# vita-epfl/CrowdNav

Measured on AMD Instinct MI355X. Metric: env-steps/sec (whole node), 4096 envs x 5 humans, ORCA step, higher is better.
Workload: dtype f32 ORCA solve + f64 env step

## Files before the change

### crowdnav_amd/csrc/crowdnav_amd.hip

```cpp
#include "engine_host.h"
#include "rollout_fused.h"
#include "records_kernels.h"

thread_local char cn_g_err[512] = "";

void cn_launch_orca(cn_engine* e, float* out_vel) {
    pick_maxl(e, [&](auto maxl) {
        pick_bool(e->P.kd, [&](auto kd) {
            hipLaunchKernelGGL((cn::orca_kernel<decltype(maxl)::value, decltype(kd)::value>), dim3(grid_envs(e)), dim3(e->P.threads),
                               e->smem, e->stream, e->P, e->S, out_vel);
        });
    });
}

extern "C" {

const char* cn_last_error(void) { return cn_g_err; }
int cn_abi_version(void) { return CN_ABI_VERSION; }

static bool headline_geometry(const cn::Params& P) {
    return P.A == 6 && P.NC == 5 && P.E == 2 && P.nA == 12 && P.pairs == 60 && P.threads == 64;
}

int cn_create(const cn_config* c, cn_engine** out) {
// ... 28 lines not shown
        return fail(CN_ERR_NO_DEVICE, "no HIP device visible: the MI355X engine has no CPU fallback");
    if (c->device < 0 || c->device >= ndev) return fail(CN_ERR_INVALID, "device %d out of range", c->device);
    CN_HIP(hipSetDevice(c->device));

    cn_engine* e = new (std::nothrow) cn_engine();
    if (!e) return fail(CN_ERR_INVALID, "out of host memory");
    e->cfg = *c;
    e->stream = nullptr;
    e->io_valid = false;
    e->steps_since_fill = -1;
    e->sarl = nullptr;
    e->orca_fresh = false;
    e->async_fill = false;
    e->rollout_done = nullptr;
    e->next_fill_stream = 0;
    for (int i = 0; i < cn_engine::kFillStreams; ++i) e->fill_streams[i] = nullptr;
    for (uint64_t& c : e->launch_counts) c = 0;
    cn::Params& P = e->P;
    P.B = c->num_envs;
    P.A = c->num_humans + 1;
    P.NC = P.A - 1;
    const int e_max = cn::kWave / P.A;
    const bool small_lp = (P.NC < c->max_neighbors ? P.NC : c->max_neighbors) <= 5;
    int e_want = env_int("CROWDNAV_AMD_ENVS_PER_WAVE", small_lp ? (P.B > 2048 ? 2 : 1) : (P.B + 4095) / 4096);
    P.E = e_want < 1 ? 1 : (e_want > e_max ? e_max : e_want);
    int w_want = env_int("CROWDNAV_AMD_WAVES_PER_BLOCK", 1);
    const int w_useful = (P.E * P.A * P.NC + cn::kWave - 1) / cn::kWave;
    if (w_want > w_useful) w_want = w_useful;
    if (w_want > cn::kMaxBlock / cn::kWave) w_want = cn::kMaxBlock / cn::kWave;
    P.threads = cn::kWave * (w_want < 1 ? 1 : w_want);
    P.nA = P.E * P.A;
    P.pairs = P.nA * P.NC;
    P.ring_depth = env_int("CROWDNAV_AMD_RING_DEPTH", 48);
    if (P.ring_depth < 1) P.ring_depth = 1;
    e->maxl = ((P.NC < c->max_neighbors ? P.NC : c->max_neighbors) <= 5) ? 5 : 10;
    P.kd = P.A > cn::kKdLeaf ? 1 : 0;
    P.sched = -1;
    e->sched_min = env_int("CROWDNAV_AMD_SCHED_MIN_STEPS", 24);
    e->sched_force = env_int("CROWDNAV_AMD_SCHED_FORCE", 0) != 0;
    e->sched_reserve = env_int("CROWDNAV_AMD_DYN_RESERVE", 0);
    e->sched_dynamic = env_int("CROWDNAV_AMD_SCHED_DYNAMIC", 1) != 0;
    e->scenario_cache = env_int("CROWDNAV_AMD_SCENARIO_CACHE", 1) != 0;
    e->dyn_visits = env_int("CROWDNAV_AMD_DYN_VISITS", 0);
    P.dyn_visits = 3;
    {
        hipDeviceProp_t prop;
        const bool ok = hipGetDeviceProperties(&prop, c->device) == hipSuccess && prop.multiProcessorCount > 0;
        e->sched_slots = 12 * (ok ? prop.multiProcessorCount : 256);
    }
    P.kdl = cn::kd_layout(P.nA, P.A, P.E);
    e->smem = cn::smem_bytes(P.nA, P.pairs, e->maxl, P.A, P.E);
    e->use_fused = env_int("CROWDNAV_AMD_FUSED", 1) != 0;
    e->fused_split = env_int("CROWDNAV_AMD_FUSED_SPLIT", 1);
    e->split_slots = 0;
    if (headline_geometry(P)) {
        int per_cu = 0;
        hipDeviceProp_t prop;
        if (hipOccupancyMaxActiveBlocksPerMultiprocessor(&per_cu, cn::rollout_fused_kernel<true, true>, 2 * cn::kWave, e->smem) == hipSuccess &&
            hipGetDeviceProperties(&prop, c->device) == hipSuccess && prop.multiProcessorCount > 0)
            e->split_slots = per_cu * prop.multiProcessorCount;
    }
    e->gen_wave = env_int("CROWDNAV_AMD_WAVE_SCENARIOS", c->num_humans > 8 ? 1 : 0) != 0;
    P.robot_visible = c->robot_visible ? 1 : 0;
    P.robot_orca = c->robot_policy == CN_ROBOT_ORCA;
    P.robot_unicycle = c->robot_kinematics == CN_UNICYCLE;
    e->async_fill = (c->flags & CN_FLAG_ASYNC_SCENARIO_FILL) != 0 && e->gen_wave;
    P.async_fill = e->async_fill ? 1 : 0;
    if (e->async_fill && !getenv("CROWDNAV_AMD_RING_DEPTH")) P.ring_depth = 144;
    e->fill_queue_wgs = env_int("CROWDNAV_AMD_FILL_QUEUE_WGS", 1024);
    P.dt = c->time_step;
    P.time_limit = c->time_limit;
    P.success_reward = c->success_reward;
    P.collision_penalty = c->collision_penalty;
    P.discomfort_dist = c->discomfort_dist;
    P.discomfort_factor = c->discomfort_penalty_factor;
    P.robot_safety = c->robot_safety_space;
    P.human_safety = c->human_safety_space;
    P.orca.neighbor_dist = (float)c->neighbor_dist;
    P.orca.inv_time_horizon = 1.0f / (float)c->time_horizon;
    P.orca.inv_time_step = 1.0f / (float)c->time_step;
    P.orca.max_neighbors = c->max_neighbors;
    e->C.num_agents = P.A;
    e->C.rule = c->scenario_rule;
    e->C.randomize = c->randomize_attributes ? 1 : 0;
    e->C.circle_radius = c->circle_radius;
    e->C.square_width = c->square_width;
    e->C.discomfort_dist = c->discomfort_dist;
    e->C.human_radius = c->human_radius;
    e->C.human_v_pref = c->human_v_pref;
    e->C.robot_radius = c->robot_radius;
    e->C.robot_v_pref = c->robot_v_pref;
    int cap_log2 = env_int("CROWDNAV_AMD_MAX_ATTEMPTS_LOG2", c->num_humans > 8 ? 23 : 20);
    if (cap_log2 < 6) cap_log2 = 6;
    if (cap_log2 > 40) cap_log2 = 40;
    e->C.max_attempts = 1ull << cap_log2;
    e->C.error = nullptr;

    const size_t n = (size_t)P.B * P.A;
    int rc = CN_OK;
    cn::StateView& S = e->S;
    if ((rc = dev_alloc(e, &S.pos, n)) || (rc = dev_alloc(e, &S.vel, n)) || (rc = dev_alloc(e, &S.goal, n)) ||
        (rc = dev_alloc(e, &S.rv, n)) || (rc = dev_alloc(e, &S.gtime, (size_t)P.B)) ||
        (rc = dev_alloc(e, &S.theta, (size_t)P.B)) ||
        (rc = dev_alloc(e, &S.rsim_radius, n)) || (rc = dev_alloc(e, &S.rsim_max_speed, (size_t)P.B)) ||
        (rc = dev_alloc(e, &S.rsim_valid, (size_t)P.B)) || (rc = dev_alloc(e, &S.mt_key, (size_t)624 * P.B)) ||
        (rc = dev_alloc(e, &S.mt_pos, (size_t)P.B)) || (rc = dev_alloc(e, &e->probe_key, (size_t)624)) ||
        (rc = dev_alloc(e, &S.ring_pos, n * P.ring_depth)) || (rc = dev_alloc(e, &S.ring_goal, n * P.ring_depth)) ||
        (rc = dev_alloc(e, &S.ring_rv, n * P.ring_depth)) ||
        (rc = dev_alloc(e, &S.ring_mt_key, e->gen_wave ? (size_t)64 : (size_t)624 * cn::kRedoLanes)) ||
        (rc = dev_alloc(e, &S.redo_list, e->gen_wave ? (size_t)1 : (size_t)P.B * P.ring_depth)) ||
        (rc = dev_alloc(e, &S.redo_count, (size_t)1)) ||
// ... 341 lines not shown
        } else {
            hipLaunchKernelGGL(cn::ring_fill_wave_async_kernel, dim3(e->P.B * e->P.ring_depth), dim3(cn::kWave), 0, fs, e->P, e->C,
                               e->S, R);
        }
        e->launch_counts[CN_COUNT_ASYNC_FILLS] += 1;
        e->steps_since_fill = 0;
        return CN_OK;
    }
    if (e->steps_since_fill >= 0 && e->steps_since_fill + n_steps <= e->P.ring_depth) {
        e->steps_since_fill += n_steps;
        return CN_OK;
    }
    const int fill_lanes = e->P.B * e->P.ring_depth;
    const dim3 fill_grid((fill_lanes + cn::kWave - 1) / cn::kWave);
    if (e->gen_wave) {
        hipLaunchKernelGGL(cn::ring_fill_wave_kernel, dim3(fill_lanes), dim3(cn::kWave), 0, e->stream, e->P, e->C, e->S, R);
    } else {
        CN_HIP(hipMemsetAsync(e->S.redo_count, 0, sizeof(int), e->stream));
        hipLaunchKernelGGL(cn::ring_fill_kernel, fill_grid, dim3(cn::kWave), 0, e->stream, e->P, e->C, e->S, R);
        hipLaunchKernelGGL(cn::ring_redo_kernel, dim3(cn::kRedoLanes / cn::kWave), dim3(cn::kWave), 0, e->stream, e->P, e->C,
                           e->S);
    }
    std::swap(e->S.ring_filled_in, e->S.ring_filled_out);
    e->launch_counts[CN_COUNT_RING_FILLS] += 1;
    e->steps_since_fill = n_steps;
    return CN_OK;
}

static int rollout_route(const cn_engine* e, const double* action) {
    const cn::Params& P = e->P;
    static const bool use_geom20 = env_int("CROWDNAV_AMD_GEOM20", 1) != 0;
    if (e->use_fused && !e->async_fill && e->maxl == 5 && !P.robot_unicycle && P.NC <= cn::kFusedMaxNC && P.pairs <= cn::kWave &&
        P.nA * 5 <= cn::kWave && P.threads == cn::kWave) {
#if defined(CN_PHASE_TIMING) || defined(CN_WAVE_TRACE)
        (void)action;
        return CN_ROUTE_FUSED;
#else
        const bool split = e->fused_split != 0 && headline_geometry(P) && P.robot_orca && action == nullptr &&
                           (grid_envs(e) <= e->split_slots || e->fused_split == 2);
        return split ? CN_ROUTE_FUSED_SPLIT : CN_ROUTE_FUSED;
#endif
    }
    if (use_geom20 && e->maxl == 10 && !P.robot_unicycle && P.A == 21 && P.NC == 20 && P.E == 1 && P.threads == 64 &&
        P.orca.max_neighbors == 10 && P.kd)
        return CN_ROUTE_SHARD;
    return CN_ROUTE_GENERIC;
}

static void launch_rollout(cn_engine* e, const cn::RolloutView& R, int n_steps, const double* action) {
    const cn::Params& P = e->P;
    const uint64_t kernels_before = e->launch_counts[CN_COUNT_ROLLOUT_KERNELS];
    const int route = rollout_route(e, action);
    if (route == CN_ROUTE_FUSED_SPLIT) {
        hipLaunchKernelGGL((cn::rollout_fused_kernel<true, true>), dim3(grid_envs(e)), dim3(2 * cn::kWave), e->smem, e->stream, e->P,
                           (const cn::StateView*)e->S_dev, (const int*)e->S.ring_filled_in, R, n_steps, action);
    } else if (route == CN_ROUTE_FUSED) {
        if (headline_geometry(P))
            hipLaunchKernelGGL((cn::rollout_fused_kernel<true>), dim3(grid_envs(e)), dim3(64), e->smem, e->stream, e->P,
                               (const cn::StateView*)e->S_dev, (const int*)e->S.ring_filled_in, R, n_steps, action);
        else
            hipLaunchKernelGGL((cn::rollout_fused_kernel<false>), dim3(grid_envs(e)), dim3(64), e->smem, e->stream, e->P,
                               (const cn::StateView*)e->S_dev, (const int*)e->S.ring_filled_in, R, n_steps, action);
    } else if (route == CN_ROUTE_SHARD) {
        const size_t smem20 = cn::smem_bytes_compact(P.nA, P.pairs, P.A, P.E);
        cn::Params Pk = e->P;
        Pk.sched = -1;
        const int slots = e->sched_slots;
        {
            const bool use_dynamic = e->sched_dynamic;
            const int reserve = e->async_fill ? e->sched_reserve : 0;
            const int G = P.B < slots - reserve ? P.B : slots - reserve;
            int visits = e->dyn_visits > 0 ? e->dyn_visits : (n_steps + 28) / 56;
            if (visits < 3) visits = 3;
            if (visits > n_steps) visits = n_steps;
            Pk.dyn_visits = visits;
            const bool helps = e->sched_force || e->async_fill || P.B > G;
            if (use_dynamic && G > 0 && n_steps >= e->sched_min && action == nullptr && helps && !e->io_host.summary &&
                !e->io_host.blocks) {
                (void)hipMemsetAsync(e->S.dyn_queue, 0, sizeof(int) * ((size_t)P.B + 1), e->stream);
                Pk.sched = cn::kSchedDynamic;
                e->launch_counts[CN_COUNT_ROLLOUT_KERNELS] += 1;
                e->launch_counts[CN_COUNT_SCHEDULED_KERNELS] += 1;
                hipLaunchKernelGGL((cn::rollout_kernel<10, false, true, true>), dim3(G), dim3(64), smem20, e->stream, Pk,
                                   (const cn::StateView*)e->S_dev, (const int*)e->S.ring_filled_in, R, n_steps, action);
                return;
            }
        }
        const int rounds_plain = (P.B + slots - 1) / slots, rounds_sched = (P.B / 4 * 3 + slots - 1) / slots;
        const bool sched = P.B % 4 == 0 && n_steps >= (e->sched_min > 48 ? e->sched_min : 48) && action == nullptr &&
                           (e->sched_force || 4 * rounds_sched < 3 * rounds_plain);
        const int q = sched ? n_steps / 3 : 0, rest = n_steps - 3 * q;
        e->launch_counts[CN_COUNT_ROLLOUT_KERNELS] += (rest > 0 ? 1 : 0) + (q > 0 ? 4 : 0);
        e->launch_counts[CN_COUNT_SCHEDULED_KERNELS] += q > 0 ? 4 : 0;
        if (rest > 0)
            hipLaunchKernelGGL((cn::rollout_kernel<10, false, true, true>), dim3(grid_envs(e)), dim3(64), smem20, e->stream, Pk,
                               (const cn::StateView*)e->S_dev, (const int*)e->S.ring_filled_in, R, rest, action);
        for (int k = 0; k < 4 && q > 0; ++k) {
            Pk.sched = k;
            hipLaunchKernelGGL((cn::rollout_kernel<10, false, true, true>), dim3(P.B / 4 * 3), dim3(64), smem20, e->stream, Pk,
                               (const cn::StateView*)e->S_dev, (const int*)e->S.ring_filled_in, R, q, action);
        }
    } else {
        pick_maxl_uni_kd(e, [&](auto maxl, auto uni, auto kd) {
            hipLaunchKernelGGL((cn::rollout_kernel<decltype(maxl)::value, decltype(uni)::value, false, decltype(kd)::value>),
                               dim3(grid_envs(e)), dim3(e->P.threads), e->smem, e->stream, e->P, (const cn::StateView*)e->S_dev,
                               (const int*)e->S.ring_filled_in, R, n_steps, action);
        });
    }
// ... 140 lines not shown
        return a;
    }();
    return &api;
}
constexpr int kNcclFloat64 = 8;
}

int cn_gather_records(cn_engine* e, void* rccl_comm, int n_ranks, int max_records, const double* blocks,
                      double* blocks_all) {
    int rc = bind(e);
    if (rc) return rc;
    if (!rccl_comm || n_ranks < 1 || max_records < 1 || !blocks || !blocks_all)
        return fail(CN_ERR_INVALID, "cn_gather_records: bad arguments");
    const RcclApi* api = rccl_api();
    if (!api->ok) return fail(CN_ERR_UNSUPPORTED, "cn_gather_records: librccl.so.1 could not be loaded");
    const size_t n = (size_t)e->P.B * cn::record_block_doubles(max_records);
    const int st = api->all_gather(blocks, blocks_all, n, kNcclFloat64, rccl_comm, e->stream);
    if (st) return fail(CN_ERR_HIP, "cn_gather_records: RCCL error %d (%s)", st, api->error_string(st));
    return CN_OK;
}

int cn_mt_random(cn_engine* e, uint32_t seed, int n, double* out) {
    int rc = bind(e);
    if (rc) return rc;
    if (n < 0 || !out) return fail(CN_ERR_INVALID, "cn_mt_random: bad arguments");
    hipLaunchKernelGGL(cn::mt_probe_kernel, dim3(1), dim3(1), 0, e->stream, e->probe_key, seed, n, out);
    CN_HIP(hipGetLastError());
    return CN_OK;
}

}

#ifdef CN_PHASE_TIMING
extern "C" int cn_debug_phase_cycles(unsigned long long* out16, int reset) {
    if (out16 && hipMemcpyFromSymbol(out16, HIP_SYMBOL(cn::cn_phase_cycles), 16 * sizeof(unsigned long long)) != hipSuccess) return -1;
    if (reset) {
        unsigned long long zero[16] = {};
        zero[13] = ~0ull;
        if (hipMemcpyToSymbol(HIP_SYMBOL(cn::cn_phase_cycles), zero, sizeof(zero)) != hipSuccess) return -1;
    }
    return 0;
}
#endif
#ifdef CN_PHASE_TIMING
extern "C" int cn_debug_lazy_counts(unsigned long long* out8, int reset) {
    if (out8 && hipMemcpyFromSymbol(out8, HIP_SYMBOL(cn::cn_lazy_counts), 16 * sizeof(unsigned long long)) != hipSuccess) return -1;
    if (reset) {
        unsigned long long zero[16] = {};
        if (hipMemcpyToSymbol(HIP_SYMBOL(cn::cn_lazy_counts), zero, sizeof(zero)) != hipSuccess) return -1;
    }
    return 0;
}
#endif
#ifdef CN_WAVE_TRACE
extern "C" int cn_debug_wave_trace(unsigned long long* out, int waves) {
    if (waves > 8192) waves = 8192;
    return hipMemcpyFromSymbol(out, HIP_SYMBOL(cn::cn_wave_trace), (size_t)waves * 6 * sizeof(unsigned long long)) == hipSuccess ? 0 : -1;
}
#endif
```

### crowdnav_amd/csrc/engine_host.h

```cpp
#pragma once
#include <hip/hip_runtime.h>

#include <cmath>
#include <cstdarg>
#include <cstdio>
#include <cstdlib>
#include <cstring>
#include <dlfcn.h>
#include <new>
#include <type_traits>
#include <utility>
#include <vector>

#include "../../include/crowdnav_amd.h"
#include "step_kernels.h"



extern thread_local char cn_g_err[512];

namespace {

[[maybe_unused]] int fail(int code, const char* fmt, ...) {
    va_list ap;
    va_start(ap, fmt);
    vsnprintf(cn_g_err, sizeof(cn_g_err), fmt, ap);
    va_end(ap);
    return code;
}

#define CN_HIP(call)                                                                              \
    do {                                                                                          \
        hipError_t err__ = (call);                                                                \
        if (err__ != hipSuccess)                                                                  \
            return fail(CN_ERR_HIP, "%s failed: %s (%s:%d)", #call, hipGetErrorString(err__), __FILE__, \
                        __LINE__);                                                                \
    } while (0)

}

struct cn_engine {
    cn_config cfg;
    cn::Params P;
    cn::ScenarioCfg C;
    cn::StateView S;
    hipStream_t stream;
    cn_rollout_io io_host;
    cn_rollout_io* io_dev;
    cn::StateView* S_dev;
    static constexpr int kFillStreams = 8;
    bool async_fill;
    hipStream_t fill_streams[kFillStreams];
    int* fill_list = nullptr;
    int fill_queue_wgs = 0;
    hipEvent_t rollout_done;
    int next_fill_stream;
    bool io_valid;
    bool rollout_begun = false;
    uint32_t begin_seed_base = 0, begin_seed_mod = 0;
    int steps_since_fill;
    struct cn_sarl* sarl;
    bool orca_fresh;
    double* discount;
    int discount_len;
    uint32_t* probe_key;
    double* summary_scratch;
    int maxl;
    bool gen_wave;
    size_t smem;
    int sched_min, sched_slots, sched_reserve, dyn_visits;
    bool sched_force, sched_dynamic;
    bool use_fused;
    int fused_split;
    int split_slots;
    bool scenario_cache;
    uint64_t launch_counts[CN_LAUNCH_COUNTERS];
    struct Slab {
        char* base;
        size_t size, used;
    };
    std::vector<Slab> slabs;
    struct AllocMark {
        std::vector<size_t> used;
    };
    AllocMark alloc_mark() const {
        AllocMark m;
        for (const Slab& s : slabs) m.used.push_back(s.used);
        return m;
    }
    void alloc_rollback(const AllocMark& m) {
        while (slabs.size() > m.used.size()) {
            (void)hipFree(slabs.back().base);
            slabs.pop_back();
        }
        for (size_t i = 0; i < slabs.size(); ++i) slabs[i].used = m.used[i];
    }
};

namespace {

constexpr size_t kSlabBytes = (size_t)32 << 20, kSlabAlign = 4096;

template <typename T>
int dev_alloc(cn_engine* e, T** out, size_t n) {
    const size_t bytes = (n * sizeof(T) + kSlabAlign - 1) / kSlabAlign * kSlabAlign;
    size_t k = 0;
    while (k < e->slabs.size() && e->slabs[k].used + bytes > e->slabs[k].size) ++k;
    if (k == e->slabs.size()) {
        const size_t size = bytes > kSlabBytes ? (bytes + ((size_t)2 << 20) - 1) >> 21 << 21 : kSlabBytes;
        void* p = nullptr;
        CN_HIP(hipMalloc(&p, size));
        e->slabs.push_back({static_cast<char*>(p), size, 0});
    }
    cn_engine::Slab& sl = e->slabs[k];
    void* p = sl.base + sl.used;
    sl.used += bytes;
    CN_HIP(hipMemset(p, 0, bytes));
    *out = static_cast<T*>(p);
    return CN_OK;
}

[[maybe_unused]] int bind(cn_engine* e) {
    if (!e) return fail(CN_ERR_INVALID, "engine is NULL");
    e->orca_fresh = false;
    CN_HIP(hipSetDevice(e->cfg.device));
    return CN_OK;
// ... 36 lines not shown
```

### crowdnav_amd/csrc/rollout_fused.h

```cpp
#pragma once
#include "step_kernels.h"

namespace cn {

constexpr int kFusedMaxNC = 5;

struct EpisodeRegs {
    double gtime;
    int state, ep_count, ring_filled;
};

template <typename T>
__device__ __forceinline__ T in_vgpr(T x) {
    asm volatile("" : "+v"(x));
    return x;
}

__device__ __forceinline__ void stage_agent(const Params& P, const Smem& s, const Lane& L, const AgentRegs& r,
                                            double human_safety) {
    if (L.lane >= P.nA) return;
    s.kin[L.lane] = make_float4((float)r.px, (float)r.py, (float)r.vx, (float)r.vy);
    s.posd[L.lane] = make_double2(r.px, r.py);
    s.rad[L.lane] = r.rad;
    s.hview[L.lane] = (float)(r.rad + 0.01 + human_safety);
// ... 34 lines not shown
        pr.my_slot = (int)((pr.row_slots >> (8 * c)) & 0xffull);
    }
    return pr;
}

template <typename Mid>
__device__ __forceinline__ void fused_pair_phase(const Params& P, const Smem& s, const PairRow& pr, float range_sq, Mid&& mid) {
    const int my_info = pr.my_info, my_slot = pr.my_slot;
    const unsigned long long row_slots = pr.row_slots;
    const int q = my_info & 0xff, c = (my_info >> 16) & 0xff;
    const int ol = (my_info >> 8) & 0xff;
    const bool robot_sim = (my_info >> 25) & 1;
    const float4 me = s.kin[q];
    const float4 other = s.kin[my_slot];
    float4 ot[kFusedMaxNC];
#pragma unroll
    for (int k = 0; k < kFusedMaxNC; ++k) ot[k] = s.kin[(int)((row_slots >> (8 * k)) & 0xffull)];
    const float* view = robot_sim ? s.rview : s.hview;
    const float rsum = view[q] + view[ol];
    const float odx = me.x - other.x, ody = me.y - other.y;
    const float mine = odx * odx + ody * ody;
    int rank = 0, within = 0;
    {
        const uint32_t mb = __float_as_uint(mine), rb = __float_as_uint(range_sq);
        uint32_t before = 0u, inside = 0u;
#pragma unroll
        for (int k = 0; k < kFusedMaxNC; ++k) {
            const float dx = me.x - ot[k].x, dy = me.y - ot[k].y;
            const uint32_t vb = __float_as_uint(dx * dx + dy * dy);
            const uint32_t tie = (uint32_t)(k - c) >> 31;
            before = __builtin_amdgcn_alignbit(before, vb - mb - tie, 31);
            inside = __builtin_amdgcn_alignbit(inside, vb - rb, 31);
        }
        within = __popc(inside);
        rank = __popc(before & inside);
    }
    mid();
    if (c == 0) s.count[q] = within < P.orca.max_neighbors ? within : P.orca.max_neighbors;
    if (mine < range_sq && rank < P.orca.max_neighbors)
        s.lines[q * kLineStride + rank] =
            make_half_plane(P.orca, me.x, me.y, me.z, me.w, other.x, other.y, other.z, other.w, rsum);
}

template <int MAXL>
__device__ __forceinline__ void fused_candidates(const Params& P, const Smem& s, int lane) {
    if (lane < P.nA * MAXL) {
        const int q = lane / MAXL, k = lane - q * MAXL;
        const float4 so = s.sol[q];
        const float4* lq = s.lines + q * kLineStride;
        s.cand2[q * kLineStride + k] = lp_line_candidate_pairs5(lq, k, lane, so.z, so.x, so.y);
    }
}

template <int MAXL, int BASE_PRIO = 0>
__device__ __forceinline__ bool fused_solve(const Params& P, const Smem& s, int lane, bool solve, float& rx, float& ry,
                                            PhaseClock* clk) {
    (void)P, (void)clk;
    rx = 0.0f, ry = 0.0f;
    int n = 0, fail = 0;
    if (solve) {
        n = s.count[lane];
        const float4 start = s.res[lane];
        rx = start.x, ry = start.y;
        fail = lp_planar_scan<MAXL>(s.lines + lane * kLineStride, s.cand2 + lane * kLineStride, n, rx, ry);
    }
    CN_TICK(clk, 3);
    const bool need = solve && fail < n;
    const unsigned long long nm = __ballot(need);
#ifdef CN_PHASE_TIMING
    if (clk) clk->acc[9] += __popcll(nm);
#endif
    if (nm == 0ull) __builtin_amdgcn_s_setprio(BASE_PRIO);
    if (nm != 0ull) {
        __builtin_amdgcn_s_setprio(3);
        constexpr int kPairs = MAXL * (MAXL - 1) / 2;
        const int n_todo = __popcll(nm);
        bool one_pass_done = false;
        if (n_todo * kPairs <= kWave) {
            const int t = lane / kPairs, m = lane - t * kPairs;
            int a = 0;
            unsigned long long rest = nm;
#pragma unroll
            for (int u = 0; u < kWave / kPairs; ++u) {
                const int bit = rest ? __ffsll((long long)rest) - 1 : 0;
                a = (u == t) ? bit : a;
                rest &= rest - 1ull;
            }
            const bool item = lane < n_todo * kPairs;
            const int i = lp3_program_of(m), base = i * (i - 1) / 2;
            const float4* la = s.lines + a * kLineStride;
            const float4 li = la[i], lj = la[m - base];
            const float radius = s.sol[a].z;
            const float4 pr = lp3_project(li, lj);
            if (item) s.proj[a * kLineStride + m] = pr;
            CN_FUSED_SYNC();
            if (item) {
                const float4* pa = s.proj + a * kLineStride + base;
                s.cand3[a * kLineStride + m] = lp_line_candidate<MAXL - 2>(pa[m - base], pa, m - base, radius, -li.w, li.z, true);
            }
            CN_FUSED_SYNC();
            if (item && m == base)
                s.cand2[a * kLineStride + i] = lp3_inner_program(s.proj + a * kLineStride, s.cand3 + a * kLineStride, i, li, radius);
            CN_FUSED_SYNC();
            if (need)
                lp3_outer_scan(s.lines + lane * kLineStride, s.cand2 + lane * kLineStride, n, fail, s.sol[lane].z, rx, ry);
            one_pass_done = true;
        } else {
            if (need) s.todo[__popcll(nm & ((1ull << lane) - 1ull))] = lane;
            CN_FUSED_SYNC();
            const int items = n_todo * kPairs;
            for (int p = lane; p < items; p += kWave) {
                const int t = p / kPairs, m = p - t * kPairs;
                const int a = s.todo[t];
                const int i = lp3_program_of(m), j = m - i * (i - 1) / 2;
                const float4* la = s.lines + a * kLineStride;
                s.proj[a * kLineStride + m] = lp3_project(la[i], la[j]);
            }
            CN_FUSED_SYNC();
            for (int p = lane; p < items; p += kWave) {
                const int t = p / kPairs, m = p - t * kPairs;
                const int a = s.todo[t];
                const int i = lp3_program_of(m), base = i * (i - 1) / 2;
                const float4 li = s.lines[a * kLineStride + i];
                const float4* pa = s.proj + a * kLineStride + base;
                s.cand3[a * kLineStride + m] = lp_line_candidate<MAXL - 2>(pa[m - base], pa, m - base, s.sol[a].z, -li.w, li.z, true);
            }
            CN_FUSED_SYNC();
        }
        if (need && !one_pass_done)
            lp3_scan(s.lines + lane * kLineStride, s.proj + lane * kLineStride, s.cand3 + lane * kLineStride, n,
                     fail, s.sol[lane].z, rx, ry);
    }
    return nm != 0ull;
}

struct StepConsts {
    double dt, limit, limit1, success, collision, ddist, dfactor, hsafety;
};
__device__ __forceinline__ StepConsts step_consts(const Params& P) {
    StepConsts K;
    K.dt = in_vgpr(P.dt), K.limit = in_vgpr(P.time_limit), K.limit1 = in_vgpr(P.time_limit - 1.0);
    K.success = in_vgpr(P.success_reward), K.collision = in_vgpr(P.collision_penalty);
    K.ddist = in_vgpr(P.discomfort_dist), K.dfactor = in_vgpr(P.discomfort_factor);
    K.hsafety = in_vgpr(P.human_safety);
    return K;
}

__device__ __forceinline__ double swept_distance(const AgentRegs& r, bool human, double2 rp, double act_x, double act_y,
                                                 double new_vx, double new_vy, double dt, double robot_rad) {
    const double x1 = r.px - rp.x, y1 = r.py - rp.y;
    const double wx = r.vx - act_x, wy = r.vy - act_y;
    const double x2 = x1 + wx * dt, y2 = y1 + wy * dt;
    const double sx = x2 - x1, sy = y2 - y1;
    double u = ((0.0 - x1) * sx + (0.0 - y1) * sy) / (sx * sx + sy * sy);
    u = (u > 1.0) ? 1.0 : ((u < 0.0) ? 0.0 : u);
    const bool degenerate = (sx == 0.0 && sy == 0.0);
    const double cx = degenerate ? 0.0 - x1 : (x1 + u * sx) - 0.0;
    const double cy = degenerate ? 0.0 - y1 : (y1 + u * sy) - 0.0;
    const double endx = r.px + new_vx * dt, endy = r.py + new_vy * dt;
    const double d = norm2(human ? cx : endx - r.gx, human ? cy : endy - r.gy);
    return human ? d - r.rad - robot_rad : d;
}

struct StepOutcome {
    double reward, dmin;
    int info;
    bool done;
};
__device__ __forceinline__ StepOutcome reduce_env(const Params& P, const Smem& s, int ebase, double gtime, const StepConsts& K) {
    const double goal_dist = s.closest[ebase];
    const double robot_rad = s.rad[ebase];
    double dmin = std::numeric_limits<double>::infinity();
    bool collision = false;
    for (int i = 1; i < P.A; ++i) {
        const double c = s.closest[ebase + i];
        const bool hit = c < 0.0;
        dmin = (!collision & !hit & (c < dmin)) ? c : dmin;
        collision = collision | hit;
    }
    const bool timeout = gtime >= K.limit1;
    const bool reaching = goal_dist < robot_rad;
    const bool danger = dmin < K.ddist;
    double reward = danger ? (dmin - K.ddist) * K.dfactor * K.dt : 0.0;
    int info = danger ? CN_DANGER : CN_NOTHING;
    reward = reaching ? K.success : reward, info = reaching ? CN_REACH_GOAL : info;
    reward = collision ? K.collision : reward, info = collision ? CN_COLLISION : info;
    reward = timeout ? 0.0 : reward, info = timeout ? CN_TIMEOUT : info;
    const bool done = timeout | collision | reaching;
    return StepOutcome{reward, dmin, info, done};
}

__device__ __forceinline__ void write_record(const cn_rollout_io& io, int env, int ep_count, int info, int cur_steps,
                                             double cur_return, double time, int cur_danger, double cur_dsum) {
    if (io.record_capacity > 0) {
        const size_t k = (size_t)env * io.record_capacity + (ep_count % io.record_capacity);
        if (io.ep_outcome) io.ep_outcome[k] = (uint8_t)info;
        if (io.ep_steps) io.ep_steps[k] = cur_steps;
        if (io.ep_return) io.ep_return[k] = cur_return;
        if (io.ep_time) io.ep_time[k] = time;
        if (io.ep_danger) io.ep_danger[k] = cur_danger;
        if (io.ep_danger_dmin_sum) io.ep_danger_dmin_sum[k] = cur_dsum;
    }
}

#ifdef CN_WAVE_TRACE
static __device__ unsigned long long cn_wave_trace[8192 * 6];
#endif

constexpr int kSplitOrcaPrio = 1;
__device__ __forceinline__ void split_barrier() {
    asm volatile("s_waitcnt lgkmcnt(0)\n\ts_barrier" ::: "memory");
}

template <int MAXL>
__device__ __forceinline__ void split_orca_wave(const Params& P, const Smem& s, int n_steps) {
    const int lane = (int)threadIdx.x - kWave;
    float2* const vel = reinterpret_cast<float2*>(s.act);
    const float range_sq = P.orca.neighbor_dist * P.orca.neighbor_dist;
    const double c_dt = in_vgpr(P.dt);
    split_barrier();
    __builtin_amdgcn_s_setprio(kSplitOrcaPrio);
    const PairRow pr = pair_row_of(P, s, lane);
    double px = 0.0, py = 0.0;
    float rx = 0.0f, ry = 0.0f;
    bool solved = false;
    for (int u = 0;;) {
        split_barrier();
        const bool ended = __builtin_amdgcn_readfirstlane(s.flag[0]) != 0;
        if (!ended) ++u;
        if (u >= n_steps) {
            split_barrier();
            break;
        }
        if (lane < P.nA) {
            if (ended) {
                const double2 p = s.posd[lane];
                px = p.x, py = p.y;
            } else if (solved) {
                px = px + (double)rx * c_dt;
                py = py + (double)ry * c_dt;
                s.kin[lane] = make_float4((float)px, (float)py, rx, ry);
            }
        }
        CN_FUSED_SYNC();
        if (lane < P.pairs) fused_pair_phase(P, s, pr, range_sq, [] {});
        split_barrier();
        fused_candidates<MAXL>(P, s, lane);
        CN_FUSED_SYNC();
        solved = lane < P.nA && s.sol[lane < P.nA ? lane : 0].w != 0.0f;
        fused_solve<MAXL, kSplitOrcaPrio>(P, s, lane, solved, rx, ry, nullptr);
        if (lane < P.nA) vel[lane] = make_float2(rx, ry);
    }
}

template <bool HEADLINE, bool SPLIT = false>
__global__ __launch_bounds__((SPLIT ? 2 : 1) * kWave, (SPLIT ? 4 : HEADLINE ? 3 : 1)) void rollout_fused_kernel(
    Params P_in, const StateView* Sd, const int* ring_filled_in, RolloutView R, int n_steps, const double* ext_action) {
    static_assert(HEADLINE || !SPLIT, "the two-wave kernel exists for the headline geometry only");
#ifdef CN_WAVE_TRACE
    const unsigned long long wt_entry = __builtin_amdgcn_s_memrealtime();
    unsigned long long wt_fallbacks = 0ull, wt_ends = 0ull;
#endif
    constexpr int MAXL = 5;
    Params P = P_in;
    if (HEADLINE) {
        P.A = 6, P.NC = 5, P.E = 2, P.nA = 12, P.pairs = 60, P.threads = 64;
    }
    const Smem s = carve<MAXL>(P);
    if constexpr (SPLIT) {
        if (__builtin_amdgcn_readfirstlane((int)threadIdx.x) >= kWave) {
            split_orca_wave<MAXL>(P, s, n_steps);
            return;
        }
    }
    const Lane L = lane_of(P);
    AgentRegs r = {};
    float robot_max_speed = 0.0f;
    const bool robot = L.valid && L.a == 0;
    const cn_rollout_io* iop = R.io;
    double theta = 0.0;
    EpisodeRegs ep{0.0, kRetired, 0, 0};
    double cur_return = 0.0, cur_dsum = 0.0;
    int cur_steps = 0, cur_danger = 0;
    {
        const StateView S = *Sd;
        const cn_rollout_io io = *iop;
        const size_t gi = L.valid ? L.gi : 0;
        const int env = L.valid ? L.env : 0;
        const double2 p0 = S.pos[gi], v0 = S.vel[gi], g0 = S.goal[gi], q0 = S.rv[gi];
        const bool have = P.robot_orca ? S.rsim_valid[env] != 0 : false;
        const float rr_kept = P.robot_orca ? S.rsim_radius[gi] : 0.0f;
        const float ms_kept = P.robot_orca ? S.rsim_max_speed[env] : 0.0f;
        const double theta0 = S.theta[env], gtime0 = S.gtime[env];
        const int state0 = io.active[env], count0 = io.ep_count[env], filled0 = ring_filled_in[env];
        const int steps0 = io.cur_steps[env];
        const double return0 = io.cur_return[env];
        const int danger0 = io.cur_danger ? io.cur_danger[env] : 0;
        const double dsum0 = io.cur_danger_dmin_sum ? io.cur_danger_dmin_sum[env] : 0.0;
        if (L.valid) {
            r.px = p0.x, r.py = p0.y, r.vx = v0.x, r.vy = v0.y, r.gx = g0.x, r.gy = g0.y, r.rad = q0.x, r.vpref = q0.y;
            ep.gtime = gtime0, ep.state = state0, ep.ep_count = count0, ep.ring_filled = filled0;
            cur_steps = steps0, cur_return = return0, cur_danger = danger0, cur_dsum = dsum0;
            if (L.a == 0) theta = theta0;
            if (P.robot_orca) {
                const float rr = have ? rr_kept : (float)(r.rad + 0.01 + P.robot_safety);
                if (!have) S.rsim_radius[L.gi] = rr;
                s.rview[L.lane] = rr;
                if (L.a == 0) {
                    robot_max_speed = have ? ms_kept : (float)r.vpref;
                    if (!have) S.rsim_max_speed[L.env] = robot_max_speed;
                }
            }
        }
    }
    build_pairs(P, s);

    if (L.valid && ep.state == kWaitingScenario && ep.ep_count < ep.ring_filled) {
        load_from_ring(P, *Sd, L, ep.ep_count % P.ring_depth, r);
        ep.state = kRunning;
        ep.gtime = 0.0;
        theta = 1.5707963267948966;
    }
    unsigned int transitions = 0;
    for (int t = threadIdx.x; t < kMaxDiscount; t += P.threads) s.disc[t] = t < R.discount_len ? R.discount[t] : 0.0;
    CN_FUSED_SYNC();
    if (L.lane == 0) s.kin[P.nA] = make_float4(std::numeric_limits<float>::infinity(), std::numeric_limits<float>::infinity(), 0.0f, 0.0f);
    const PairRow pr = pair_row_of(P, s, L.lane);
    const StepConsts K = step_consts(P);
    stage_agent(P, s, L, r, K.hsafety);
    CN_FUSED_SYNC();

#ifdef CN_PHASE_TIMING
    PhaseClock clock = {};
    PhaseClock* clk = &clock;
    clock.last = __builtin_readcyclecounter();
#else
    PhaseClock* clk = nullptr;
    (void)clk;
#endif
    const float range_sq = P.orca.neighbor_dist * P.orca.neighbor_dist;
#ifdef CN_WAVE_TRACE
    const unsigned long long wt_loop = __builtin_amdgcn_s_memrealtime();
#endif
    if constexpr (SPLIT) {
        float2* const vel = reinterpret_cast<float2*>(s.act);
        if (L.lane == 0) s.flag[0] = 1;
        split_barrier();
        bool skip = true;
        for (int u = 0;;) {
            split_barrier();
            if (!skip) ++u;
            const bool running = L.valid && ep.state == kRunning;
            const AgentRegs r0 = r;
            double act_x = 0.0, act_y = 0.0, new_vx = 0.0, new_vy = 0.0;
            if (!skip && L.lane < P.nA) {
                const float2 mine = vel[L.lane], robots = vel[L.ebase];
                act_x = (double)robots.x, act_y = (double)robots.y;
                new_vx = (L.a == 0) ? act_x : (double)mine.x;
                new_vy = (L.a == 0) ? act_y : (double)mine.y;
                if (running) {
                    r.px = r.px + new_vx * K.dt;
                    r.py = r.py + new_vy * K.dt;
                    r.vx = new_vx;
                    r.vy = new_vy;
                }
            }
            if (u < n_steps && L.lane < P.nA) {
                float4 sol4, start4;
                preferred_velocity(r, (L.a == 0) ? robot_max_speed : (float)r.vpref, running && (L.a > 0 || P.robot_orca), sol4, start4);
                s.sol[L.lane] = sol4;
                s.res[L.lane] = start4;
            }
            split_barrier();
            bool ended = false;
            if (!skip) {
                const double2 rp = make_double2(__shfl(r0.px, L.ebase), __shfl(r0.py, L.ebase));
                if (L.valid) s.closest[L.lane] = swept_distance(r0, L.a > 0, rp, act_x, act_y, new_vx, new_vy, K.dt, s.rad[L.ebase]);
                CN_FUSED_SYNC();
                bool done = false;
                if (running) {
                    const double disc_t = s.disc[cur_steps < kMaxDiscount ? cur_steps : kMaxDiscount - 1];
                    const StepOutcome o = reduce_env(P, s, L.ebase, ep.gtime, K);
                    done = o.done;
                    ep.gtime += K.dt;
                    ++transitions;
                    cur_return = cur_return + (cur_steps < kMaxDiscount ? disc_t : 0.0) * o.reward;
                    ++cur_steps;
                    cur_danger += o.info == CN_DANGER ? 1 : 0;
                    cur_dsum = o.info == CN_DANGER ? cur_dsum + o.dmin : cur_dsum;
                    if (done) {
                        const cn_rollout_io io = *iop;
                        const StateView S = *Sd;
                        AgentRegs next = r;
                        load_from_ring(P, S, L, (ep.ep_count + 1) % P.ring_depth, next);
                        if (L.a == 0) write_record(io, L.env, ep.ep_count, o.info, cur_steps, cur_return, (o.info == CN_TIMEOUT) ? K.limit : ep.gtime, cur_danger, cur_dsum);
                        cur_steps = 0, cur_return = 0.0, cur_danger = 0, cur_dsum = 0.0;
                        ++ep.ep_count;
                        ep.gtime = 0.0;
                        const int64_t c = episode_id(io, L.env, ep.ep_count);
                        if (io.episode_limit >= 0 && c >= io.episode_limit) {
                            ep.state = kRetired;
                        } else if (ep.ep_count < ep.ring_filled) {
                            r = next;
                            theta = 1.5707963267948966;
                        } else {
                            ep.state = kWaitingScenario;
                        }
                    }
                }
                ended = __ballot(done) != 0ull;
            }
            if (ended) stage_agent(P, s, L, r, K.hsafety);
            if (L.lane == 0) s.flag[0] = ended ? 1 : 0;
            skip = ended;
            if (u >= n_steps) break;
        }
    }
    const int one_wave_steps = SPLIT ? 0 : n_steps;
    for (int step = 0; step < one_wave_steps; ++step) {
        const bool running = L.valid && ep.state == kRunning;
        const bool solve = running && (L.a > 0 || P.robot_orca);

        if (L.lane < P.pairs) {
            float4 sol4, start4;
            fused_pair_phase(P, s, pr, range_sq, [&] {
                preferred_velocity(r, (L.a == 0) ? robot_max_speed : (float)r.vpref, solve, sol4, start4);
            });
            if (L.lane < P.nA) {
                s.sol[L.lane] = sol4;
                s.res[L.lane] = start4;
            }
        }
        CN_FUSED_SYNC();
        CN_TICK(clk, 2);

        fused_candidates<MAXL>(P, s, L.lane);
        CN_FUSED_SYNC();

        float rx, ry;
        const bool fell_back = fused_solve<MAXL>(P, s, L.lane, solve, rx, ry, clk);
        (void)fell_back;
#ifdef CN_WAVE_TRACE
        if (fell_back) ++wt_fallbacks;
#endif
        CN_TICK(clk, 8);

        double act_x, act_y;
        if (P.robot_orca) {
            act_x = (double)__shfl(rx, L.ebase);
            act_y = (double)__shfl(ry, L.ebase);
        } else {
            act_x = L.valid ? ext_action[2 * (size_t)L.env] : 0.0;
            act_y = L.valid ? ext_action[2 * (size_t)L.env + 1] : 0.0;
        }
        const double new_vx = (L.a == 0) ? act_x : (double)rx;
        const double new_vy = (L.a == 0) ? act_y : (double)ry;

        if (L.valid)
            s.closest[L.lane] = swept_distance(r, L.a > 0, s.posd[L.ebase], act_x, act_y, new_vx, new_vy, K.dt, s.rad[L.ebase]);
        CN_FUSED_SYNC();
        CN_TICK(clk, 5);

        if (running) {
            const double disc_t = s.disc[cur_steps < kMaxDiscount ? cur_steps : kMaxDiscount - 1];
            const StepOutcome o = reduce_env(P, s, L.ebase, ep.gtime, K);
            const double reward = o.reward, dmin = o.dmin;
            const int info = o.info;
            const bool done = o.done;
            ep.gtime += K.dt;
            r.px = r.px + new_vx * K.dt;
            r.py = r.py + new_vy * K.dt;
            r.vx = new_vx;
            r.vy = new_vy;
            ++transitions;
            cur_return = cur_return + (cur_steps < kMaxDiscount ? disc_t : 0.0) * reward;
            ++cur_steps;
            cur_danger += info == CN_DANGER ? 1 : 0;
            cur_dsum = info == CN_DANGER ? cur_dsum + dmin : cur_dsum;
#ifdef CN_WAVE_TRACE
            if (__ballot(done) != 0ull) ++wt_ends;
#endif
            if (done) {
                const cn_rollout_io io = *iop;
                if (L.a == 0) write_record(io, L.env, ep.ep_count, info, cur_steps, cur_return, (info == CN_TIMEOUT) ? K.limit : ep.gtime, cur_danger, cur_dsum);
                cur_steps = 0, cur_return = 0.0, cur_danger = 0, cur_dsum = 0.0;
                ++ep.ep_count;
                ep.gtime = 0.0;
                const int64_t c = episode_id(io, L.env, ep.ep_count);
                if (io.episode_limit >= 0 && c >= io.episode_limit) {
                    ep.state = kRetired;
                } else if (ep.ep_count < ep.ring_filled) {
                    load_from_ring(P, *Sd, L, ep.ep_count % P.ring_depth, r);
                    theta = 1.5707963267948966;
// ... 59 lines not shown
```

Measured before the change: 1.394 billion.

## Let env wave speculatively compute LP3 head for predicted fallback agents in split kernel

In the two-wave split kernel, the ORCA wave publishes which agents needed the LP3 fallback last step, and the env wave uses that mask as a prediction. It computes the LP3 projection and candidate head for those agents in parallel with the ORCA wave's line building, at raised priority. When the current fallback set falls within the prediction, the ORCA wave skips recomputing the head. This adds an extra barrier on steps that have a prediction, and the work is wasted when the prediction misses. It also adds an optional compile-time probe for barrier wait accounting.

```diff
diff --git a/crowdnav_amd/csrc/crowdnav_amd.hip b/crowdnav_amd/csrc/crowdnav_amd.hip
--- a/crowdnav_amd/csrc/crowdnav_amd.hip
+++ b/crowdnav_amd/csrc/crowdnav_amd.hip
@@ -104,11 +104,14 @@
     e->smem = cn::smem_bytes(P.nA, P.pairs, e->maxl, P.A, P.E);
     e->use_fused = env_int("CROWDNAV_AMD_FUSED", 1) != 0;
     e->fused_split = env_int("CROWDNAV_AMD_FUSED_SPLIT", 1);
+    e->split_assist = env_int("CROWDNAV_AMD_SPLIT_ASSIST", 1) != 0 ? cn::kAssistHead : 0;
     e->split_slots = 0;
     if (headline_geometry(P)) {
         int per_cu = 0;
         hipDeviceProp_t prop;
-        if (hipOccupancyMaxActiveBlocksPerMultiprocessor(&per_cu, cn::rollout_fused_kernel<true, true>, 2 * cn::kWave, e->smem) == hipSuccess &&
+        const bool head = (e->split_assist & cn::kAssistHead) != 0;
+        if ((head ? hipOccupancyMaxActiveBlocksPerMultiprocessor(&per_cu, cn::rollout_fused_kernel<true, true, cn::kAssistHead>, 2 * cn::kWave, e->smem)
+                  : hipOccupancyMaxActiveBlocksPerMultiprocessor(&per_cu, cn::rollout_fused_kernel<true, true>, 2 * cn::kWave, e->smem)) == hipSuccess &&
             hipGetDeviceProperties(&prop, c->device) == hipSuccess && prop.multiProcessorCount > 0)
             e->split_slots = per_cu * prop.multiProcessorCount;
     }
@@ -556,8 +559,12 @@
     const uint64_t kernels_before = e->launch_counts[CN_COUNT_ROLLOUT_KERNELS];
     const int route = rollout_route(e, action);
     if (route == CN_ROUTE_FUSED_SPLIT) {
-        hipLaunchKernelGGL((cn::rollout_fused_kernel<true, true>), dim3(grid_envs(e)), dim3(2 * cn::kWave), e->smem, e->stream, e->P,
-                           (const cn::StateView*)e->S_dev, (const int*)e->S.ring_filled_in, R, n_steps, action);
+        if (e->split_assist & cn::kAssistHead)
+            hipLaunchKernelGGL((cn::rollout_fused_kernel<true, true, cn::kAssistHead>), dim3(grid_envs(e)), dim3(2 * cn::kWave), e->smem,
+                               e->stream, e->P, (const cn::StateView*)e->S_dev, (const int*)e->S.ring_filled_in, R, n_steps, action);
+        else
+            hipLaunchKernelGGL((cn::rollout_fused_kernel<true, true>), dim3(grid_envs(e)), dim3(2 * cn::kWave), e->smem, e->stream, e->P,
+                               (const cn::StateView*)e->S_dev, (const int*)e->S.ring_filled_in, R, n_steps, action);
     } else if (route == CN_ROUTE_FUSED) {
         if (headline_geometry(P))
             hipLaunchKernelGGL((cn::rollout_fused_kernel<true>), dim3(grid_envs(e)), dim3(64), e->smem, e->stream, e->P,
@@ -804,6 +811,16 @@
     return 0;
 }
 #endif
+#ifdef CN_SPLIT_PROBE
+extern "C" int cn_debug_split_probe(unsigned long long* out32, int reset) {
+    if (out32 && hipMemcpyFromSymbol(out32, HIP_SYMBOL(cn::cn_split_probe), 32 * sizeof(unsigned long long)) != hipSuccess) return -1;
+    if (reset) {
+        unsigned long long zero[32] = {};
+        if (hipMemcpyToSymbol(HIP_SYMBOL(cn::cn_split_probe), zero, sizeof(zero)) != hipSuccess) return -1;
+    }
+    return 0;
+}
+#endif
 #ifdef CN_WAVE_TRACE
 extern "C" int cn_debug_wave_trace(unsigned long long* out, int waves) {
     if (waves > 8192) waves = 8192;
diff --git a/crowdnav_amd/csrc/engine_host.h b/crowdnav_amd/csrc/engine_host.h
--- a/crowdnav_amd/csrc/engine_host.h
+++ b/crowdnav_amd/csrc/engine_host.h
@@ -72,6 +72,7 @@
     bool sched_force, sched_dynamic;
     bool use_fused;
     int fused_split;
+    int split_assist;
     int split_slots;
     bool scenario_cache;
     uint64_t launch_counts[CN_LAUNCH_COUNTERS];
diff --git a/crowdnav_amd/csrc/rollout_fused.h b/crowdnav_amd/csrc/rollout_fused.h
--- a/crowdnav_amd/csrc/rollout_fused.h
+++ b/crowdnav_amd/csrc/rollout_fused.h
@@ -110,9 +110,61 @@
     }
 }
 
-template <int MAXL, int BASE_PRIO = 0>
-__device__ __forceinline__ bool fused_solve(const Params& P, const Smem& s, int lane, bool solve, float& rx, float& ry,
-                                            PhaseClock* clk) {
+__device__ __forceinline__ void split_barrier() {
+    asm volatile("s_waitcnt lgkmcnt(0)\n\ts_barrier" ::: "memory");
+}
+
+struct Lp3Item {
+    int a, m, i, base;
+    bool item;
+    float4 li, lj;
+    float radius;
+};
+template <int MAXL>
+__device__ __forceinline__ Lp3Item lp3_item_of(const Smem& s, int lane, unsigned long long mask) {
+    constexpr int kPairs = MAXL * (MAXL - 1) / 2;
+    Lp3Item it;
+    const int t = lane / kPairs;
+    it.m = lane - t * kPairs;
+    it.a = 0;
+    unsigned long long rest = mask;
+#pragma unroll
+    for (int u = 0; u < kWave / kPairs; ++u) {
+        const int bit = rest ? __ffsll((long long)rest) - 1 : 0;
+        it.a = (u == t) ? bit : it.a;
+        rest &= rest - 1ull;
+    }
+    it.item = lane < (int)__popcll(mask) * kPairs;
+    it.i = lp3_program_of(it.m), it.base = it.i * (it.i - 1) / 2;
+    const float4* la = s.lines + it.a * kLineStride;
+    it.li = la[it.i], it.lj = la[it.m - it.base];
+    it.radius = s.sol[it.a].z;
+    return it;
+}
+template <int MAXL>
+__device__ __forceinline__ void lp3_head(const Smem& s, const Lp3Item& it) {
+    const float4 pr = lp3_project(it.li, it.lj);
+    if (it.item) s.proj[it.a * kLineStride + it.m] = pr;
+    CN_FUSED_SYNC();
+    if (it.item) {
+        const float4* pa = s.proj + it.a * kLineStride + it.base;
+        s.cand3[it.a * kLineStride + it.m] =
+            lp_line_candidate<MAXL - 2>(pa[it.m - it.base], pa, it.m - it.base, it.radius, -it.li.w, it.li.z, true);
+    }
+}
+
+template <int MAXL>
+__device__ __forceinline__ bool split_has_head(unsigned int pred, int u, int n_steps) {
+    return pred != 0u && __popc(pred) * (MAXL * (MAXL - 1) / 2) <= kWave && u < n_steps;
+}
+
+struct NoOp {
+    __device__ __forceinline__ void operator()() const {}
+};
+template <int MAXL, int BASE_PRIO = 0, typename AfterScan = NoOp>
+__device__ __forceinline__ unsigned long long fused_solve(const Params& P, const Smem& s, int lane, bool solve, float& rx,
+                                                          float& ry, PhaseClock* clk, unsigned long long have = 0ull,
+                                                          AfterScan&& after_scan = NoOp{}) {
     (void)P, (void)clk;
     rx = 0.0f, ry = 0.0f;
     int n = 0, fail = 0;
@@ -128,6 +180,7 @@
 #ifdef CN_PHASE_TIMING
     if (clk) clk->acc[9] += __popcll(nm);
 #endif
+    after_scan();
     if (nm == 0ull) __builtin_amdgcn_s_setprio(BASE_PRIO);
     if (nm != 0ull) {
         __builtin_amdgcn_s_setprio(3);
@@ -135,28 +188,16 @@
         const int n_todo = __popcll(nm);
         bool one_pass_done = false;
         if (n_todo * kPairs <= kWave) {
-            const int t = lane / kPairs, m = lane - t * kPairs;
-            int a = 0;
-            unsigned long long rest = nm;
-#pragma unroll
-            for (int u = 0; u < kWave / kPairs; ++u) {
-                const int bit = rest ? __ffsll((long long)rest) - 1 : 0;
-                a = (u == t) ? bit : a;
-                rest &= rest - 1ull;
-            }
-            const bool item = lane < n_todo * kPairs;
-            const int i = lp3_program_of(m), base = i * (i - 1) / 2;
-            const float4* la = s.lines + a * kLineStride;
-            const float4 li = la[i], lj = la[m - base];
-            const float radius = s.sol[a].z;
-            const float4 pr = lp3_project(li, lj);
-            if (item) s.proj[a * kLineStride + m] = pr;
-            CN_FUSED_SYNC();
-            if (item) {
-                const float4* pa = s.proj + a * kLineStride + base;
-                s.cand3[a * kLineStride + m] = lp_line_candidate<MAXL - 2>(pa[m - base], pa, m - base, radius, -li.w, li.z, true);
-            }
-            CN_FUSED_SYNC();
+            const Lp3Item it = lp3_item_of<MAXL>(s, lane, nm);
+            const bool item = it.item;
+            const int a = it.a, i = it.i, m = it.m, base = it.base;
+            const float4 li = it.li;
+            const float radius = it.radius;
+            const bool hit = (nm & ~have) == 0ull;
+            if (!hit) {
+                lp3_head<MAXL>(s, it);
+                CN_FUSED_SYNC();
+            }
             if (item && m == base)
                 s.cand2[a * kLineStride + i] = lp3_inner_program(s.proj + a * kLineStride, s.cand3 + a * kLineStride, i, li, radius);
             CN_FUSED_SYNC();
@@ -189,7 +230,7 @@
             lp3_scan(s.lines + lane * kLineStride, s.proj + lane * kLineStride, s.cand3 + lane * kLineStride, n,
                      fail, s.sol[lane].z, rx, ry);
     }
-    return nm != 0ull;
+    return nm;
 }
 
 struct StepConsts {
@@ -266,11 +307,61 @@
 #endif
 
 constexpr int kSplitOrcaPrio = 1;
-__device__ __forceinline__ void split_barrier() {
-    asm volatile("s_waitcnt lgkmcnt(0)\n\ts_barrier" ::: "memory");
-}
-
-template <int MAXL>
+constexpr int kAssistHead = 1;
+#ifndef CN_SPLIT_HEAD_PRIO
+#define CN_SPLIT_HEAD_PRIO 2
+#endif
+#ifndef CN_SPLIT_HEAD_TAIL_PRIO
+#define CN_SPLIT_HEAD_TAIL_PRIO 1
+#endif
+
+#ifdef CN_SPLIT_PROBE
+constexpr bool kSplitProbe = true;
+static __device__ unsigned long long cn_split_probe[32];
+#define SPLIT_PROBE_DECL()                                                                                   \
+    unsigned long long sp_cnt[7] = {}, sp_wait[3] = {}, sp_w1[2] = {}, sp_n1[2] = {}, sp_dt = 0ull; \
+    bool sp_prev_head = false
+#define SPLIT_PROBE_WAIT(k, barrier)                                   \
+    do {                                                               \
+        const unsigned long long sp_t0 = __builtin_readcyclecounter(); \
+        barrier;                                                       \
+        sp_dt = __builtin_readcyclecounter() - sp_t0;                  \
+        sp_wait[k] += sp_dt;                                           \
+    } while (0)
+#define SPLIT_PROBE_AFTER_1(word, head)                               \
+    do {                                                               \
+        if ((word) != 0u) sp_w1[0] += sp_dt, ++sp_n1[0];               \
+        if (sp_prev_head) sp_w1[1] += sp_dt, ++sp_n1[1];               \
+        sp_prev_head = (head);                                         \
+    } while (0)
+#define SPLIT_PROBE_STEP(ended, nm, head, pred)                                  \
+    do {                                                                         \
+        const bool sp_hit = (head) && (nm) != 0ull && ((nm) & ~(unsigned long long)(pred)) == 0ull; \
+        ++sp_cnt[0], sp_cnt[1] += (ended) ? 1 : 0, sp_cnt[2] += (nm) != 0ull ? 1 : 0, sp_cnt[3] += (head) ? 1 : 0; \
+        sp_cnt[4] += sp_hit ? 1 : 0, sp_cnt[5] += ((nm) != 0ull && !sp_hit) ? 1 : 0, sp_cnt[6] += ((head) && (nm) == 0ull) ? 1 : 0; \
+    } while (0)
+#define SPLIT_PROBE_FLUSH(lane, base)                                                        \
+    do {                                                                                     \
+        if ((lane) == 0) {                                                                   \
+            if ((base) == 0)                                                                 \
+                for (int k = 0; k < 7; ++k) atomicAdd(&cn_split_probe[k], sp_cnt[k]);        \
+            for (int k = 0; k < 3; ++k) atomicAdd(&cn_split_probe[((base) ? 10 : 7) + k], sp_wait[k]); \
+            for (int k = 0; k < 2; ++k) {                                                    \
+                atomicAdd(&cn_split_probe[((base) ? 17 : 13) + k], sp_w1[k]);                \
+                atomicAdd(&cn_split_probe[((base) ? 19 : 15) + k], sp_n1[k]);                \
+            }                                                                                \
+        }                                                                                    \
+    } while (0)
+#else
+constexpr bool kSplitProbe = false;
+#define SPLIT_PROBE_DECL() (void)0
+#define SPLIT_PROBE_WAIT(k, barrier) barrier
+#define SPLIT_PROBE_AFTER_1(word, head) (void)0
+#define SPLIT_PROBE_STEP(ended, nm, head, pred) (void)0
+#define SPLIT_PROBE_FLUSH(lane, base) (void)0
+#endif
+
+template <int MAXL, int ASSIST>
 __device__ __forceinline__ void split_orca_wave(const Params& P, const Smem& s, int n_steps) {
     const int lane = (int)threadIdx.x - kWave;
     float2* const vel = reinterpret_cast<float2*>(s.act);
@@ -282,14 +373,18 @@
     double px = 0.0, py = 0.0;
     float rx = 0.0f, ry = 0.0f;
     bool solved = false;
+    SPLIT_PROBE_DECL();
     for (int u = 0;;) {
-        split_barrier();
+        SPLIT_PROBE_WAIT(0, split_barrier());
         const bool ended = __builtin_amdgcn_readfirstlane(s.flag[0]) != 0;
+        const unsigned int pred = ((ASSIST & kAssistHead) || kSplitProbe) ? (unsigned int)__builtin_amdgcn_readfirstlane(s.flag[1]) : 0u;
         if (!ended) ++u;
         if (u >= n_steps) {
             split_barrier();
             break;
         }
+        const bool head = (ASSIST & kAssistHead) ? split_has_head<MAXL>(pred, u, n_steps) : false;
+        SPLIT_PROBE_AFTER_1(pred, head);
         if (lane < P.nA) {
             if (ended) {
                 const double2 p = s.posd[lane];
@@ -302,19 +397,25 @@
         }
         CN_FUSED_SYNC();
         if (lane < P.pairs) fused_pair_phase(P, s, pr, range_sq, [] {});
-        split_barrier();
+        SPLIT_PROBE_WAIT(1, split_barrier());
         fused_candidates<MAXL>(P, s, lane);
         CN_FUSED_SYNC();
         solved = lane < P.nA && s.sol[lane < P.nA ? lane : 0].w != 0.0f;
-        fused_solve<MAXL, kSplitOrcaPrio>(P, s, lane, solved, rx, ry, nullptr);
+        const unsigned long long nm = fused_solve<MAXL, kSplitOrcaPrio>(P, s, lane, solved, rx, ry, nullptr, head ? pred : 0u, [&] {
+            if (head) SPLIT_PROBE_WAIT(2, split_barrier());
+        });
         if (lane < P.nA) vel[lane] = make_float2(rx, ry);
-    }
-}
-
-template <bool HEADLINE, bool SPLIT = false>
+        if (((ASSIST & kAssistHead) || kSplitProbe) && lane == 0) s.flag[1] = (int)nm;
+        SPLIT_PROBE_STEP(ended, nm, head, pred);
+    }
+    SPLIT_PROBE_FLUSH(lane, 0);
+}
+
+template <bool HEADLINE, bool SPLIT = false, int ASSIST = 0>
 __global__ __launch_bounds__((SPLIT ? 2 : 1) * kWave, (SPLIT ? 4 : HEADLINE ? 3 : 1)) void rollout_fused_kernel(
     Params P_in, const StateView* Sd, const int* ring_filled_in, RolloutView R, int n_steps, const double* ext_action) {
     static_assert(HEADLINE || !SPLIT, "the two-wave kernel exists for the headline geometry only");
+    static_assert(SPLIT || ASSIST == 0, "the env wave assists an ORCA wave: two-wave kernel only");
 #ifdef CN_WAVE_TRACE
     const unsigned long long wt_entry = __builtin_amdgcn_s_memrealtime();
     unsigned long long wt_fallbacks = 0ull, wt_ends = 0ull;
@@ -327,7 +428,7 @@
     const Smem s = carve<MAXL>(P);
     if constexpr (SPLIT) {
         if (__builtin_amdgcn_readfirstlane((int)threadIdx.x) >= kWave) {
-            split_orca_wave<MAXL>(P, s, n_steps);
+            split_orca_wave<MAXL, ASSIST>(P, s, n_steps);
             return;
         }
     }
@@ -402,12 +503,15 @@
 #endif
     if constexpr (SPLIT) {
         float2* const vel = reinterpret_cast<float2*>(s.act);
-        if (L.lane == 0) s.flag[0] = 1;
+        if (L.lane == 0) s.flag[0] = 1, s.flag[1] = 0;
         split_barrier();
         bool skip = true;
+        SPLIT_PROBE_DECL();
         for (int u = 0;;) {
-            split_barrier();
+            SPLIT_PROBE_WAIT(0, split_barrier());
             if (!skip) ++u;
+            const unsigned int pred = ((ASSIST & kAssistHead) || kSplitProbe) ? (unsigned int)__builtin_amdgcn_readfirstlane(s.flag[1]) : 0u;
+            SPLIT_PROBE_AFTER_1(pred, (ASSIST & kAssistHead) != 0 && split_has_head<MAXL>(pred, u, n_steps));
             const bool running = L.valid && ep.state == kRunning;
             const AgentRegs r0 = r;
             double act_x = 0.0, act_y = 0.0, new_vx = 0.0, new_vy = 0.0;
@@ -429,7 +533,16 @@
                 s.sol[L.lane] = sol4;
                 s.res[L.lane] = start4;
             }
-            split_barrier();
+            SPLIT_PROBE_WAIT(1, split_barrier());
+            if constexpr ((ASSIST & kAssistHead) != 0) {
+                if (split_has_head<MAXL>(pred, u, n_steps)) {
+                    __builtin_amdgcn_s_setprio(CN_SPLIT_HEAD_PRIO);
+                    const Lp3Item it = lp3_item_of<MAXL>(s, L.lane, (unsigned long long)pred);
+                    lp3_head<MAXL>(s, it);
+                    __builtin_amdgcn_s_setprio(CN_SPLIT_HEAD_TAIL_PRIO);
+                    SPLIT_PROBE_WAIT(2, split_barrier());
+                }
+            }
             bool ended = false;
             if (!skip) {
                 const double2 rp = make_double2(__shfl(r0.px, L.ebase), __shfl(r0.py, L.ebase));
@@ -471,8 +584,10 @@
             if (ended) stage_agent(P, s, L, r, K.hsafety);
             if (L.lane == 0) s.flag[0] = ended ? 1 : 0;
             skip = ended;
+            if constexpr ((ASSIST & kAssistHead) != 0 && CN_SPLIT_HEAD_TAIL_PRIO != 0) __builtin_amdgcn_s_setprio(0);
             if (u >= n_steps) break;
         }
+        SPLIT_PROBE_FLUSH(L.lane, 10);
     }
     const int one_wave_steps = SPLIT ? 0 : n_steps;
     for (int step = 0; step < one_wave_steps; ++step) {
@@ -496,7 +611,7 @@
         CN_FUSED_SYNC();
 
         float rx, ry;
-        const bool fell_back = fused_solve<MAXL>(P, s, L.lane, solve, rx, ry, clk);
+        const bool fell_back = fused_solve<MAXL>(P, s, L.lane, solve, rx, ry, clk) != 0ull;
         (void)fell_back;
 #ifdef CN_WAVE_TRACE
         if (fell_back) ++wt_fallbacks;
```

Measured after the change: 1.414 billion, median of 6. 1.4% higher.
